# Krabbens/edge-diffusion-tts

Hardware: AMD Instinct MI355X
Metric: mel-frames/sec (whole node), 4-step DDIM, hidden=160 L=4, B=256 T=512 (higher is better)
Workload: dtype f32

## Files before the change

edge-diffusion-tts_amd/csrc/edtts_device.h:

```cpp
#pragma once
#include <hip/hip_runtime.h>
#include <stdint.h>
#include <type_traits>

#if !defined(EDTTS_EXPERIMENTS) && (                                                                                               \
    defined(EDTTS_ABLATE_QKVSTORES) || defined(EDTTS_ABLATE_KVLOADS) || defined(EDTTS_DIAG) || defined(EDTTS_KV2) ||                \
    defined(EDTTS_H_DMA) || defined(EDTTS_SPLITLOAD) || defined(EDTTS_STAMPS) || defined(EDTTS_DS_ABL) ||                           \
    defined(EDTTS_FAST_BUILD) || defined(EDTTS_W2) || defined(EDTTS_WAVELOG) || defined(EDTTS_PIN_MASK) || defined(EDTTS_HANDOVER) || defined(EDTTS_DS_BURST) || defined(EDTTS16_MFMA_SUM) || defined(EDTTS_DS_STAMPS) || defined(EDTTS_TAIL_RING2) || defined(EDTTS_RB) || defined(EDTTS_WMAX) ||        \
    defined(EDTTS_STAMP_THREAD) || defined(EDTTS_STAMP_HEAD) ||                                                                     \
    defined(EDTTS16_ABLATE_BARRIER) || defined(EDTTS16_ABLATE_DMA) || defined(EDTTS16_PHASES) || defined(EDTTS16_NF) ||             \
    defined(EDTTS16_W1) || defined(EDTTS16_QLDS) || defined(EDTTS16_KVDEPTH) || defined(EDTTS16_IMG) || defined(EDTTS16_HP) ||      \
    defined(EDTTS16_EVEN_STEPS))
#error "tuning / ablation / diagnostic / measured-and-rejected variant switches are scratch-only: add -DEDTTS_EXPERIMENTS"
#endif

#ifndef EDTTS_PIN_MASK
#define EDTTS_PIN_MASK 0x4
#endif
#ifndef EDTTS_W2
#define EDTTS_W2 0
#endif
#if EDTTS_W2
#define EDTTS_PIN_ACC(x) asm volatile("" : "+v"(x))
#else
#define EDTTS_PIN_ACC(x) asm volatile("" : "+a"(x))
#endif
typedef float f4 __attribute__((ext_vector_type(4)));
typedef float f2 __attribute__((ext_vector_type(2)));

#define EDTTS_MFMA(a, b, c) __builtin_amdgcn_mfma_f32_16x16x4f32((a), (b), (c), 0, 0, 0)
#define EDTTS_DEV __device__ __forceinline__

#ifdef EDTTS_STAMPS
#define STAMP_SEL_HEAD(sel) ((sel) & 0xff)
#define STAMPX(p, i, sel) do { if ((p) && (int)blockIdx.x == ((sel) >> 16) && (int)threadIdx.x == 64 * (((sel) >> 8) & 0xff)) (p)[i] = __builtin_amdgcn_s_memtime(); } while (0)
#else
#define STAMPX(p, i, sel) do { } while (0)
#endif

namespace edtts {

constexpr int kCtxWaves = 4;

template <int H_, int HEADS_, int MEL_, int NF_ = 2>
struct Cfg {
  static constexpr int H = H_, HEADS = HEADS_, MEL = MEL_, NF = NF_;
  static constexpr int WF = 16 * NF;
  static constexpr int QT = NF >= 2 ? 2 : 1;
  static constexpr int NHALF = NF / QT;
  static constexpr int DH = H / HEADS;
  static constexpr int DFULL = DH / 16;
  static constexpr int DREM = DH % 16;
  static constexpr int DT = (DH + 15) / 16;
  static constexpr int DHP = DT * 16;
  static constexpr int HT = H / 16;
  static constexpr int MT = MEL / 16;
  static constexpr int R = H / 2, RT = R / 16;
  static constexpr int VR = (HEADS - 1) * DH + DHP;
#ifndef EDTTS_WMAX
#define EDTTS_WMAX 2
#endif
  static constexpr int WAVES0 = (HT * NF * 4 <= 160) ? 4 : 2;
  static constexpr int WAVES = NF == 1 ? 1 : (WAVES0 < EDTTS_WMAX ? WAVES0 : EDTTS_WMAX);
  static constexpr bool Q_IN_LDS = !(EDTTS_W2 && NF == 2) && WF * H * 4 * 2 <= 40 * 1024;
  static constexpr int THREADS = 64 * WAVES;
  static constexpr bool DEFER = EDTTS_W2 && NF == 2 && H == 160;
  static constexpr int OHEAD_BYTES = DFULL * NF * 1024 + (DREM ? NF * 512 : 0);
  static_assert(NF == 1 || NF == 2 || NF == 4, "frame tiles per wave");
  static_assert(H % 32 == 0 && MEL % 16 == 0 && H % HEADS == 0, "dims");
  static_assert(DREM == 0 || DREM == 8, "head_dim % 16 must be 0 or 8");
};

EDTTS_DEV f4 splat(float v) { return f4{v, v, v, v}; }
EDTTS_DEV f4 ldg4(const float* p) { return *reinterpret_cast<const f4*>(p); }
EDTTS_DEV f2 ldg2(const float* p) { return *reinterpret_cast<const f2*>(p); }
EDTTS_DEV void stg4(float* p, f4 v) { *reinterpret_cast<f4*>(p) = v; }
EDTTS_DEV f4 ldg4_sbase(const float* base, unsigned byte_off) {
  return *reinterpret_cast<const f4*>(reinterpret_cast<const char*>(base) + byte_off);
}
EDTTS_DEV f2 ldg2_sbase(const float* base, unsigned byte_off) {
  return *reinterpret_cast<const f2*>(reinterpret_cast<const char*>(base) + byte_off);
}

template <int NT, int NF>
EDTTS_DEV void dma_tile_to_lds(const float* src, int ld, f4* lds_wave) {
  typedef __attribute__((address_space(3))) char* lds_char_t;
  const unsigned base = __builtin_amdgcn_readfirstlane((unsigned)(size_t)(lds_char_t)(char*)lds_wave);
#pragma unroll
  for (int nt = 0; nt < NT; ++nt)
#pragma unroll
    for (int ft = 0; ft < NF; ++ft) {
      const float* p = src + 16 * nt + (size_t)ft * 16 * ld;
      asm volatile("s_mov_b32 m0, %1\n\ts_nop 0\n\tglobal_load_lds_dwordx4 %0, off" ::"v"(p), "s"(base + (unsigned)(nt * NF + ft) * 1024u) : "m0", "memory");
    }
}

typedef unsigned u4v __attribute__((ext_vector_type(4)));
typedef unsigned u2v __attribute__((ext_vector_type(2)));
EDTTS_DEV __amdgpu_buffer_rsrc_t make_rsrc(const void* base) {
  return __builtin_amdgcn_make_buffer_rsrc(const_cast<void*>(base), 0, 0xFFFFFFFF, 0x00020000);
}
EDTTS_DEV f4 bufld4(__amdgpu_buffer_rsrc_t r, unsigned voff, unsigned soff) {
  return __builtin_bit_cast(f4, __builtin_amdgcn_raw_buffer_load_b128(r, voff, soff, 0));
}
EDTTS_DEV f2 bufld2(__amdgpu_buffer_rsrc_t r, unsigned voff, unsigned soff) {
  return __builtin_bit_cast(f2, __builtin_amdgcn_raw_buffer_load_b64(r, voff, soff, 0));
}

EDTTS_DEV float sqrt_rn(float x) { return (float)sqrt((double)x); }
EDTTS_DEV float div_rn(float a, float b) { return (float)((double)a / (double)b); }

EDTTS_DEV float group_sum(float v) {
  unsigned u = __float_as_uint(v);
  auto a = __builtin_amdgcn_permlane16_swap(u, u, false, false);
  v = __uint_as_float(a[0]) + __uint_as_float(a[1]);
  u = __float_as_uint(v);
  auto b = __builtin_amdgcn_permlane32_swap(u, u, false, false);
  return __uint_as_float(b[0]) + __uint_as_float(b[1]);
}
EDTTS_DEV float group_max(float v) {
  unsigned u = __float_as_uint(v);
  auto a = __builtin_amdgcn_permlane16_swap(u, u, false, false);
  v = fmaxf(__uint_as_float(a[0]), __uint_as_float(a[1]));
  u = __float_as_uint(v);
  auto b = __builtin_amdgcn_permlane32_swap(u, u, false, false);
  return fmaxf(__uint_as_float(b[0]), __uint_as_float(b[1]));
}
EDTTS_DEV float hsum(f4 v) { return (v[0] + v[1]) + (v[2] + v[3]); }
EDTTS_DEV float hmax(f4 v) { return fmaxf(fmaxf(v[0], v[1]), fmaxf(v[2], v[3])); }

#ifndef EDTTS_RB
#define EDTTS_RB 2
#endif
constexpr int kRefillBurst = EDTTS_RB;
template <int RN>
struct FragRing {
  static constexpr int RN_ = RN;
  __amdgpu_buffer_rsrc_t rs;
  unsigned soff;
  unsigned voff;
  f4 r[RN];
  EDTTS_DEV f4 frag(int i) const {
    return bufld4(rs, voff, soff + (unsigned)i * 1024u);
  }
  EDTTS_DEV void prime(const float* base, int lane) {
    rs = make_rsrc(base);
    soff = 0;
    voff = (unsigned)lane * 16u;
#pragma unroll
    for (int i = 0; i < RN; ++i) r[i] = frag(i);
  }
  EDTTS_DEV const f4& at(int i) const { return r[i % RN]; }
  EDTTS_DEV void refill(int lo, int hi) {
#pragma unroll
    for (int i = lo; i < hi; ++i) r[i % RN] = frag(i + RN);
    __builtin_amdgcn_sched_barrier(0);
  }
  template <int N>
  EDTTS_DEV void refill_after(int i) {
    constexpr int B = kRefillBurst < RN ? kRefillBurst : RN;
    if ((i + 1) % B == 0) refill(i + 1 - B, i + 1);
    else if (i == N - 1) refill(N - N % B, N);
  }
  EDTTS_DEV void advance(int n) { soff += (unsigned)n * 1024u; }
};

template <int KT, int RN, int NF>
EDTTS_DEV void gemm_phase(FragRing<RN>& ring, const f4 (&in)[KT][NF], f4 (&acc)[NF]) {
  static_assert(KT % RN == 0, "phase length must be a multiple of the ring size");
  constexpr bool SPLIT = NF < 4;
  f4 b[NF];
  if (SPLIT) {
#pragma unroll
    for (int ft = 0; ft < NF; ++ft) b[ft] = splat(0.f);
  }
#pragma unroll
  for (int kt = 0; kt < KT; ++kt) {
    const f4& a = ring.at(kt);
#pragma unroll
    for (int r = 0; r < 4; ++r)
#pragma unroll
      for (int ft = 0; ft < NF; ++ft) {
        if (SPLIT && (kt & 1)) b[ft] = EDTTS_MFMA(a[r], in[kt][ft][r], b[ft]);
        else acc[ft] = EDTTS_MFMA(a[r], in[kt][ft][r], acc[ft]);
      }
    ring.template refill_after<KT>(kt);
  }
  if (SPLIT) {
#pragma unroll
    for (int ft = 0; ft < NF; ++ft) acc[ft] += b[ft];
  }
  ring.advance(KT);
}

template <int KT, int RN, int NF>
EDTTS_DEV void gemm_phase_pair(FragRing<RN>& ring, const f4 (&in)[KT][NF], f4 (&a)[NF], f4 (&b)[NF]) {
  static_assert((2 * KT) % RN == 0, "phase length must be a multiple of the ring size");
#pragma unroll
  for (int kt = 0; kt < KT; ++kt) {
    const f4& fa = ring.at(2 * kt);
    const f4& fb = ring.at(2 * kt + 1);
#pragma unroll
    for (int r = 0; r < 4; ++r) {
#pragma unroll
      for (int ft = 0; ft < NF; ++ft) a[ft] = EDTTS_MFMA(fa[r], in[kt][ft][r], a[ft]);
#pragma unroll
      for (int ft = 0; ft < NF; ++ft) b[ft] = EDTTS_MFMA(fb[r], in[kt][ft][r], b[ft]);
    }
    ring.template refill_after<2 * KT>(2 * kt);
    ring.template refill_after<2 * KT>(2 * kt + 1);
  }
  ring.advance(2 * KT);
}

template <int NT, int RN, int NF, int NR = 4>
EDTTS_DEV void ktile_phase(FragRing<RN>& ring, const f4 (&in)[NF], f4 (&acc)[NT][NF]) {
  static_assert(NT % RN == 0, "phase length must be a multiple of the ring size");
  constexpr int STEP = NF < 4 ? 2 : 1;
#pragma unroll
  for (int nt = 0; nt < NT; nt += STEP) {
#pragma unroll
    for (int r = 0; r < NR; ++r)
#pragma unroll
      for (int u = 0; u < STEP; ++u)
        if (nt + u < NT) {
          const f4& fa = ring.at(nt + u);
#pragma unroll
          for (int ft = 0; ft < NF; ++ft) acc[nt + u][ft] = EDTTS_MFMA(fa[r], in[ft][r], acc[nt + u][ft]);
        }
#pragma unroll
    for (int u = 0; u < STEP; ++u)
      if (nt + u < NT) ring.template refill_after<NT>(nt + u);
  }
  ring.advance(NT);
}

template <int NT, int NF>
EDTTS_DEV void rms_norm_tile(const f4 (&x)[NT][NF], const float* __restrict__ w, const float* __restrict__ mod, int g,
                             f4 (&y)[NT][NF]) {
  constexpr int N = NT * 16;
  float rs[NF];
#pragma unroll
  for (int ft = 0; ft < NF; ++ft) {
    float ss = 0.f;
#pragma unroll
    for (int t = 0; t < NT; ++t) ss += hsum(x[t][ft] * x[t][ft]);
    rs[ft] = rsqrtf(group_sum(ss) * (1.0f / N) + 1e-6f);
  }
#pragma unroll
  for (int t = 0; t < NT; ++t) {
    const f4 wv = ldg4(w + 16 * t + 4 * g);
    f4 sc = splat(1.f), sh = splat(0.f);
    if (mod != nullptr) {
      sc = ldg4(mod + 16 * t + 4 * g);
      sh = ldg4(mod + N + 16 * t + 4 * g);
    }
#pragma unroll
    for (int ft = 0; ft < NF; ++ft) {
      f4 a = x[t][ft] * rs[ft] * wv;
// ... 658 lines not shown
```

edge-diffusion-tts_amd/csrc/edtts_kernels.hip:

```cpp
#include <hip/hip_runtime.h>
#include <math.h>
#include <stdarg.h>
#include <stdlib.h>
#include <stdio.h>
#include <string.h>

#include "../../include/edtts.h"
#include "edtts_device.h"

using namespace edtts;

static thread_local char g_err[512] = "";
static int fail(int code, const char* fmt, ...) __attribute__((format(printf, 2, 3)));
static int fail(int code, const char* fmt, ...) {
  va_list ap;
  va_start(ap, fmt);
  vsnprintf(g_err, sizeof(g_err), fmt, ap);
  va_end(ap);
  return code;
}
#define HIP_TRY(expr)                                                                                   \
  do {                                                                                                  \
    hipError_t e_ = (expr);                                                                             \
    if (e_ != hipSuccess) return fail(EDTTS_ERR_HIP, "%s failed: %s", #expr, hipGetErrorString(e_));    \
// ... 318 lines not shown
  const int64_t* step_idx;
  int use_host, host_has_step;
  int t_host[kMaxHostRows], step_host[kMaxHostRows];
  int H, L, n_step;
  const float *freqs, *t1T, *t1b, *t3T, *t3b, *step;
  const float* blob;
  unsigned ada1T[kMaxLayers], ada1b[kMaxLayers], ada3T[kMaxLayers], ada3b[kMaxLayers];
  float* cond;
  float* tcond;
  unsigned* err;
};
__global__ __launch_bounds__(256) void k_cond_mlp(CondArgs a) {
  extern __shared__ float sm[];
  float* e = sm;
  float* u = sm + a.H;
  const int row = blockIdx.x, tid = threadIdx.x, H = a.H, half = H / 2;
  const float tf = a.use_host ? (float)a.t_host[row] : (float)a.t[row];
  for (int j = tid; j < H; j += blockDim.x) {
    const float arg = tf * a.freqs[j < half ? j : j - half];
    e[j] = j < half ? sinf(arg) : cosf(arg);
  }
  __syncthreads();
  for (int n = tid; n < H; n += blockDim.x) {
    float acc = a.t1b[n];
#pragma unroll 8
    for (int k = 0; k < H; ++k) acc = fmaf(e[k], a.t1T[(size_t)k * H + n], acc);
    u[n] = 0.5f * acc * (1.0f + erff(acc * 0.70710678118654752440f));
  }
  __syncthreads();
  long sidx = -1;
  if (a.use_host ? a.host_has_step : (a.step_idx != nullptr)) {
    sidx = a.use_host ? (long)a.step_host[row] : (long)a.step_idx[row];
    if (sidx < 0 || sidx >= a.n_step) {
      if (tid == 0) atomicOr(a.err, (unsigned)EDTTS_IDX_STEP);
      sidx = sidx < 0 ? 0 : a.n_step - 1;
    }
  }
  for (int n = tid; n < H; n += blockDim.x) {
    float acc = a.t3b[n];
#pragma unroll 8
    for (int k = 0; k < H; ++k) acc = fmaf(u[k], a.t3T[(size_t)k * H + n], acc);
    if (sidx >= 0) acc += a.step[(size_t)sidx * H + n];
    a.tcond[(size_t)row * H + n] = acc;
  }
}
__global__ __launch_bounds__(256) void k_cond_ada(CondArgs a) {
  extern __shared__ float sm[];
  const int row = blockIdx.x, lw = blockIdx.y, l = lw >> 1, which = lw & 1, H = a.H;
  for (int k = threadIdx.x; k < H; k += blockDim.x) sm[k] = a.tcond[(size_t)row * H + k];
  __syncthreads();
  const float* WT = a.blob + (which ? a.ada3T[l] : a.ada1T[l]);
  const float* bb = a.blob + (which ? a.ada3b[l] : a.ada1b[l]);
  float* out = a.cond + (((size_t)row * a.L + l) * 2 + which) * 2 * H;
  for (int n = blockIdx.z * blockDim.x + threadIdx.x; n < 2 * H; n += gridDim.z * blockDim.x) {
    float acc = bb[n];
#pragma unroll 8
    for (int k = 0; k < H; ++k) acc = fmaf(sm[k], WT[(size_t)k * 2 * H + n], acc);
    out[n] = n < H ? 1.0f + acc : acc;
  }
}

struct KArgs {
  int B, T, Tp, S, Sp, window, max_pos, max_cpos, n_tok, SD, L;
  const float* x;
  float* h;
  const float *q, *k, *vT;
  float *q_out, *k_out, *vT_out;
  float *kc, *vcT;
  const void* unused_[3];
  const int64_t* sem_idx;
  const float* sem_feat;
  const float* cond;
  int cond_bstride;
  int layer;
  int ffn_tiles;
  int diag_skip;
  unsigned long long* stamps;
  const float *tok, *semp, *semp_b, *cpe, *inp, *inp_b, *pe;
  const float *n1w, *proj_b, *n2w, *n3w, *up_b, *down_b, *fnw, *fnb, *outp_b;
  const float* stream;
  float *eps, *x_prev, *x0;
  float c_s1m, c_sab, c_sabp, c_dir;
  float p_coef1, p_coef2, p_sd;
  const float* noise;
  unsigned long long seed;
  unsigned long long philox_base;
  unsigned step;
  LmsCoef lms;
  VpredCoef vp;
  const float* v_uncond;
  const float *h_new, *h_old;
  float *x0_hist, *x0_all;
  const int64_t *t_len, *s_len;
  int t_dbl;
};

EDTTS_DEV int utt_len_of(int64_t v, int full, bool dbl) {
  const int hi = dbl ? full >> 1 : full;
  const int n = v < 1 ? 1 : (v > hi ? hi : (int)v);
  return dbl ? 2 * n : n;
}
EDTTS_DEV int utt_len(const int64_t* len, int b, int full, bool dbl = false) {
  if (len == nullptr) return full;
  return utt_len_of(len[__builtin_amdgcn_readfirstlane(b)], full, dbl);
}
EDTTS_DEV int utt_len_lane(const int64_t* len, int b, int full, bool dbl = false) {
  return len == nullptr ? full : utt_len_of(len[b], full, dbl);
}
EDTTS_DEV int live_end(int n) { return (n + 31) & ~31; }

EDTTS_DEV int remap_block(int bid, int nblk) {
  const int q = nblk >> 3, r = nblk & 7, xcd = bid & 7, idx = bid >> 3;
  const int base = xcd < r ? xcd * (q + 1) : r * (q + 1) + (xcd - r) * q;
  return base + idx;
}

struct TileId {
  int b, m0;
  bool valid;
};
EDTTS_DEV TileId wave_tile(int B, int Tp, int waves_per_block, int wave_frames) {
  const int wave = __builtin_amdgcn_readfirstlane(threadIdx.x >> 6);
  const int tpu = Tp / wave_frames;
  int w = remap_block(blockIdx.x, gridDim.x) * waves_per_block + wave;
  TileId t;
  t.valid = w < B * tpu;
  w = t.valid ? w : B * tpu - 1;
  t.b = w / tpu;
  t.m0 = (w - t.b * tpu) * wave_frames;
  return t;
}

#ifndef EDTTS_TAIL_RING2
#define EDTTS_TAIL_RING2 1
#endif
template <class C>
EDTTS_DEV void qkv_tail(WStream<C>& ring0, const f4 (&hn)[C::HT][C::NF], const KArgs& a, int b, int m0, int lane) {
  constexpr int NF = C::NF;
  static_assert(C::HT % 2 == 0, "hidden must be a multiple of 32 (n-tile pairs)");
#if EDTTS_TAIL_RING2
  constexpr int RN0 = WStream<C>::RN_;
  static_assert((2 * C::HT) % (2 * RN0) == 0, "a pair phase must be a whole number of turns of the doubled ring");
  FragRing<2 * RN0> ring;
  ring.rs = ring0.rs; ring.soff = ring0.soff; ring.voff = ring0.voff;
#pragma unroll
  for (int i = 0; i < RN0; ++i) ring.r[i] = ring0.at(i);
#pragma unroll
  for (int i = RN0; i < 2 * RN0; ++i) ring.r[i] = ring.frag(i);
  __builtin_amdgcn_sched_barrier(0);
#else
  WStream<C>& ring = ring0;
#endif
  const int fq = lane & 15, g = lane >> 4;
  const size_t rowbase = (size_t)b * a.Tp + m0 + fq;
#pragma unroll
  for (int which = 0; which < 3; ++which) {
    for (int nt = 0; nt < C::HT; nt += 2) {
      f4 acc[2][NF];
#pragma unroll
      for (int ft = 0; ft < NF; ++ft) acc[0][ft] = acc[1][ft] = splat(0.f);
      gemm_phase_pair<C::HT>(ring, hn, acc[0], acc[1]);
#ifdef EDTTS_ABLATE_QKVSTORES
      if (a.T > 0) continue;
#endif
#pragma unroll
      for (int u = 0; u < 2; ++u) {
        if (which < 2) {
          float* dst = (which == 0 ? a.q_out : a.k_out) + rowbase * C::H + 16 * (nt + u) + 4 * g;
#pragma unroll
          for (int ft = 0; ft < NF; ++ft) {
            __builtin_nontemporal_store(acc[u][ft], reinterpret_cast<f4*>(dst + (size_t)ft * 16 * C::H));
          }
        } else {
          float* dst = a.vT_out + ((size_t)b * C::VR + 16 * (nt + u) + 4 * g) * a.Tp + m0 + fq;
#pragma unroll
          for (int r = 0; r < 4; ++r)
#pragma unroll
            for (int ft = 0; ft < NF; ++ft) {
              __builtin_nontemporal_store(acc[u][ft][r], dst + (size_t)r * a.Tp + 16 * ft);
            }
        }
      }
    }
  }
}

template <class C>
__global__ __launch_bounds__(C::THREADS) void k_prologue(KArgs a) {
  constexpr int NF = C::NF;
  const TileId tl = wave_tile(a.B, a.Tp, C::WAVES, C::WF);
  if (!tl.valid) return;
  const int lane = threadIdx.x & 63, fq = lane & 15, g = lane >> 4;
  const int b = tl.b, m0 = tl.m0;
  const int Tb = utt_len(a.t_len, b, a.T, a.t_dbl);
  if (m0 >= live_end(Tb)) return;
  WStream<C> ring;
  ring.prime(a.stream, lane);
  f4 xin[C::MT][NF];
#pragma unroll
  for (int ft = 0; ft < NF; ++ft) {
    const int f = m0 + 16 * ft + fq;
#pragma unroll
    for (int t = 0; t < C::MT; ++t)
      xin[t][ft] = f < Tb ? ldg4(a.x + ((size_t)b * a.T + f) * C::MEL + 16 * t + 4 * g) : splat(0.f);
  }
  f4 h[C::HT][NF];
#pragma unroll
  for (int nt = 0; nt < C::HT; ++nt) {
    const f4 bias = ldg4(a.inp_b + 16 * nt + 4 * g);
#pragma unroll
    for (int ft = 0; ft < NF; ++ft) h[nt][ft] = bias;
  }
  {
    constexpr int N = C::HT * C::MT;
    static_assert(N % WStream<C>::RN_ == 0 && C::HT % 2 == 0, "in_proj must be a whole number of ring turns");
#pragma unroll
    for (int nt = 0; nt < C::HT; nt += 2)
#pragma unroll
      for (int kt = 0; kt < C::MT; ++kt) {
        const int i = nt * C::MT + 2 * kt;
        const f4& fa = ring.at(i);
        const f4& fb = ring.at(i + 1);
#pragma unroll
        for (int r = 0; r < 4; ++r) {
#pragma unroll
          for (int ft = 0; ft < NF; ++ft) h[nt][ft] = EDTTS_MFMA(fa[r], xin[kt][ft][r], h[nt][ft]);
#pragma unroll
          for (int ft = 0; ft < NF; ++ft) h[nt + 1][ft] = EDTTS_MFMA(fb[r], xin[kt][ft][r], h[nt + 1][ft]);
        }
        ring.template refill_after<N>(i);
        ring.template refill_after<N>(i + 1);
      }
    ring.advance(N);
  }
#pragma unroll
  for (int ft = 0; ft < NF; ++ft) {
    int f = m0 + 16 * ft + fq;
    f = f < a.max_pos ? f : a.max_pos - 1;
#pragma unroll
    for (int nt = 0; nt < C::HT; ++nt) h[nt][ft] += ldg4(a.pe + (size_t)f * C::H + 16 * nt + 4 * g);
  }
  {
    float* hp = a.h + ((size_t)b * a.Tp + m0 + fq) * C::H + 4 * g;
#pragma unroll
    for (int nt = 0; nt < C::HT; ++nt)
#pragma unroll
      for (int ft = 0; ft < NF; ++ft) stg4(hp + 16 * nt + (size_t)ft * 16 * C::H, h[nt][ft]);
  }
  f4 hn[C::HT][NF];
  const float* mod = a.cond + (size_t)b * a.cond_bstride;
  rms_norm_tile<C::HT, NF>(h, a.n1w, mod, g, hn);
  qkv_tail<C>(ring, hn, a, b, m0, lane);
}

enum { TAIL_QKV = 0, TAIL_EPS = 1, TAIL_DDIM = 2, TAIL_DDPM = 3, TAIL_LMS = 4, TAIL_VPRED = 5 };

template <int TAIL>
EDTTS_DEV void tail_apply(const KArgs& a, size_t idx, f4 ev) {
  if (TAIL == TAIL_EPS) {
    stg4(a.eps + idx, ev);
  } else if (TAIL == TAIL_LMS) {
    const f4 xv = ldg4(a.x + idx);
    f4 hn = splat(0.f), ho = splat(0.f);
    if (a.lms.mode >= 2) hn = ldg4(a.h_new + idx);
    if (a.lms.mode >= 3) ho = ldg4(a.h_old + idx);
    f4 x0, xn;
#pragma unroll
    for (int r = 0; r < 4; ++r) {
      float v0, vn;
      lms_elem(xv[r], ev[r], hn[r], ho[r], a.lms, v0, vn);
      x0[r] = v0;
      xn[r] = vn;
    }
    stg4(a.x0_hist + idx, x0);
    if (a.x0_all) stg4(a.x0_all + idx, x0);
    stg4(a.x_prev + idx, xn);
  } else if (TAIL == TAIL_VPRED) {
    const bool guided = a.v_uncond != nullptr;
    const f4 xv = ldg4(a.x + idx);
    const f4 vu = ldg4((guided ? a.v_uncond : a.x) + idx);
    f4 v, xn;
#pragma unroll
    for (int r = 0; r < 4; ++r) v[r] = guided ? cfg_combine(ev[r], vu[r], a.vp.cfg) : ev[r];
#pragma unroll
    for (int r = 0; r < 4; ++r) xn[r] = vpred_elem(xv[r], v[r], a.vp);
    stg4(a.x_prev + idx, xn);
  } else if (TAIL == TAIL_DDPM) {
    const f4 xv = ldg4(a.x + idx);
    const f4 nz = a.noise ? ldg4(a.noise + idx) : philox_normal4(a.seed, a.step, (a.philox_base + idx) >> 2);
    const DdpmCoef cf{a.p_coef1, a.p_coef2, a.p_sd};
    f4 xp;
#pragma unroll
    for (int r = 0; r < 4; ++r) xp[r] = ddpm_elem(xv[r], ev[r], nz[r], cf);
    stg4(a.x_prev + idx, xp);
  } else {
    const f4 xv = ldg4(a.x + idx);
    f4 x0, xp;
#pragma unroll
    for (int r = 0; r < 4; ++r) {
      float v0, vp;
      ddim_elem(xv[r], ev[r], a.c_s1m, a.c_sab, a.c_sabp, a.c_dir, v0, vp);
      x0[r] = v0;
      xp[r] = vp;
    }
    stg4(a.x0 + idx, x0);
    stg4(a.x_prev + idx, xp);
  }
}
template <int TAIL>
EDTTS_DEV void tail_zero(const KArgs& a, size_t idx) {
  const f4 z = splat(0.f);
  if (TAIL == TAIL_EPS) {
    stg4(a.eps + idx, z);
  } else if (TAIL == TAIL_LMS) {
    stg4(a.x0_hist + idx, z);
    if (a.x0_all) stg4(a.x0_all + idx, z);
    stg4(a.x_prev + idx, z);
  } else if (TAIL == TAIL_DDIM) {
    stg4(a.x0 + idx, z);
    stg4(a.x_prev + idx, z);
  } else {
    stg4(a.x_prev + idx, z);
  }
}
template <int TAIL>
EDTTS_DEV void tail_store(const KArgs& a, int f, int Tb, size_t idx, f4 ev) {
  if (f < Tb) tail_apply<TAIL>(a, idx, ev);
  else tail_zero<TAIL>(a, idx);
}

struct QGlobal {
  __amdgpu_buffer_rsrc_t rs;
  unsigned v4, v2;
  int H;
  EDTTS_DEV QGlobal(const float* row_m0, int H_, int fq, int g) : rs(make_rsrc(row_m0)), v4((unsigned)(fq * H_ + 4 * g) * 4u), v2((unsigned)(fq * H_ + 2 * g) * 4u), H(H_) {}
  EDTTS_DEV f4 q4(int ft, int col) const { return bufld4(rs, v4, (unsigned)(ft * 16 * H + col) * 4u); }
  EDTTS_DEV f2 q2(int ft, int col) const { return bufld2(rs, v2, (unsigned)(ft * 16 * H + col) * 4u); }
};
struct QLds {
  const float* b4;
  const float* b2;
  int ld;
  EDTTS_DEV QLds(const float* tile, int ld_, int fq, int g) : b4(tile + fq * ld_ + 4 * g), b2(tile + fq * ld_ + 2 * g), ld(ld_) {}
  EDTTS_DEV f4 q4(int ft, int col) const { return *reinterpret_cast<const f4*>(b4 + ft * 16 * ld + col); }
  EDTTS_DEV f2 q2(int ft, int col) const { return *reinterpret_cast<const f2*>(b2 + ft * 16 * ld + col); }
};

template <class C, int TAIL>
EDTTS_DEV void layer_tile(const KArgs& a, float* smem, int wave, int lane, int b, int m0, int Tb, int Sb) {
  constexpr int NF = C::NF;
  const int fq = lane & 15, g = lane >> 4;
  f4* const stash = reinterpret_cast<f4*>(smem) + (size_t)wave * C::HT * NF * 64 + lane;
  char* const obuf = reinterpret_cast<char*>(smem) + (size_t)wave * C::HT * NF * 1024;
  static_assert(!C::DEFER || C::HEADS * C::OHEAD_BYTES <= C::HT * NF * 1024, "attention outputs must fit the wave's parking place");
  constexpr int QLDS = C::H;
  float* qtile = smem + (size_t)C::WAVES * C::HT * NF * 256 + (size_t)wave * C::WF * QLDS;
  const size_t rowbase = (size_t)b * a.Tp + m0 + fq;

  STAMPX(a.stamps, 0, a.diag_skip);
  WStream<C> ring;
  ring.prime(a.stream, lane);

  f4 h[C::HT][NF];
  float* const hp = a.h + rowbase * C::H + 4 * g;
  auto park_h = [&]() {
#pragma unroll
    for (int nt = 0; nt < C::HT; ++nt)
#pragma unroll
      for (int ft = 0; ft < NF; ++ft) stash[(nt * NF + ft) * 64] = h[nt][ft];
  };
  auto add_parked_h = [&]() {
#pragma unroll
    for (int nt = 0; nt < C::HT; ++nt)
#pragma unroll
      for (int ft = 0; ft < NF; ++ft) h[nt][ft] += stash[(nt * NF + ft) * 64];
  };
#ifdef EDTTS_DIAG
#define DIAG_ON(bit) (!(a.diag_skip & (bit)))
#else
#define DIAG_ON(bit) true
#endif
  {
#ifndef EDTTS_H_DMA
#define EDTTS_H_DMA 0
#endif
#if EDTTS_H_DMA
    dma_tile_to_lds<C::HT, NF>(hp, C::H, reinterpret_cast<f4*>(smem) + (size_t)wave * C::HT * NF * 64);
#else
    if constexpr (!C::DEFER) {
#pragma unroll
      for (int nt = 0; nt < C::HT; ++nt)
#pragma unroll
        for (int ft = 0; ft < NF; ++ft) h[nt][ft] = ldg4(hp + 16 * nt + (size_t)ft * 16 * C::H);
      park_h();
    }
#endif
    auto init_proj_bias = [&]() {
#pragma unroll
      for (int nt = 0; nt < C::HT; ++nt) {
        const f4 pb = ldg4(a.proj_b + 16 * nt + 4 * g);
#pragma unroll
        for (int ft = 0; ft < NF; ++ft) h[nt][ft] = pb;
      }
    };
    if constexpr (!C::DEFER) init_proj_bias();
    if (DIAG_ON(1)) {
      QGlobal ql(a.q + ((size_t)b * a.Tp + m0) * C::H, C::H, fq, g);
      attention_fused<C, true, C::DEFER ? O_DEFER : O_FUSED>(ql, a.k + (size_t)b * a.Tp * C::H, a.vT + (size_t)b * C::VR * a.Tp, a.Tp, Tb, a.window, m0,
                               lane, ring, h, obuf, init_proj_bias, a.stamps ? a.stamps + 8 : nullptr, a.diag_skip);
    }
    if constexpr (C::DEFER) {
#pragma unroll
      for (int nt = 0; nt < C::HT; ++nt)
#pragma unroll
        for (int ft = 0; ft < NF; ++ft) h[nt][ft] += ldg4(hp + 16 * nt + (size_t)ft * 16 * C::H);
    } else {
      add_parked_h();
    }
    STAMPX(a.stamps, 1, a.diag_skip);
  }
  if (DIAG_ON(2)) {
    {
      f4 hn[C::HT][NF];
      rms_norm_tile<C::HT, NF>(h, a.n2w, nullptr, g, hn);
      if constexpr (C::DEFER) {
#pragma unroll
        for (int nt = 0; nt < C::HT; ++nt)
#pragma unroll
          for (int ft = 0; ft < NF; ++ft) stg4(hp + 16 * nt + (size_t)ft * 16 * C::H, h[nt][ft]);
      } else {
        park_h();
      }
      for (int nt = 0; nt < C::HT; nt += 2) {
        f4 acc[2][NF];
#pragma unroll
        for (int ft = 0; ft < NF; ++ft) acc[0][ft] = acc[1][ft] = splat(0.f);
        gemm_phase_pair<C::HT>(ring, hn, acc[0], acc[1]);
#pragma unroll
        for (int u = 0; u < 2; ++u)
#pragma unroll
          for (int ft = 0; ft < NF; ++ft) {
            if (C::Q_IN_LDS) stg4(qtile + (16 * ft + fq) * QLDS + 16 * (nt + u) + 4 * g, acc[u][ft]);
            else stg4(const_cast<float*>(a.q) + (rowbase + 16 * ft) * C::H + 16 * (nt + u) + 4 * g, acc[u][ft]);
          }
      }
    }
    STAMPX(a.stamps, 2, a.diag_skip);
    auto zero_h = [&]() {
#pragma unroll
      for (int nt = 0; nt < C::HT; ++nt)
#pragma unroll
        for (int ft = 0; ft < NF; ++ft) h[nt][ft] = splat(0.f);
    };
    if constexpr (!C::DEFER) zero_h();
    if constexpr (C::Q_IN_LDS) {
      QLds ql(qtile, QLDS, fq, g);
      attention_fused<C, false, C::DEFER ? O_DEFER : O_FUSED>(ql, a.kc + (size_t)b * a.Sp * C::H, a.vcT + (size_t)b * C::VR * a.Sp, a.Sp, Sb, -1, m0, lane,
                                ring, h, obuf, zero_h, a.stamps ? a.stamps + 40 : nullptr, a.diag_skip);
    } else {
      QGlobal ql(a.q + ((size_t)b * a.Tp + m0) * C::H, C::H, fq, g);
      attention_fused<C, false, C::DEFER ? O_DEFER : O_FUSED>(ql, a.kc + (size_t)b * a.Sp * C::H, a.vcT + (size_t)b * C::VR * a.Sp, a.Sp, Sb, -1, m0, lane,
                                ring, h, obuf, zero_h);
    }
    if constexpr (C::DEFER) {
#pragma unroll
      for (int nt = 0; nt < C::HT; ++nt)
#pragma unroll
        for (int ft = 0; ft < NF; ++ft) h[nt][ft] += ldg4(hp + 16 * nt + (size_t)ft * 16 * C::H);
    } else {
      add_parked_h();
    }
    STAMPX(a.stamps, 3, a.diag_skip);
  }
  if (DIAG_ON(4)) {
    f4 hn[C::HT][NF];
    const float* mod = a.cond + (size_t)b * a.cond_bstride + ((size_t)a.layer * 2 + 1) * 2 * C::H;
    rms_norm_tile<C::HT, NF>(h, a.n3w, mod, g, hn);
    park_h();
#pragma unroll
    for (int nt = 0; nt < C::HT; ++nt) {
      const f4 db = ldg4(a.down_b + 16 * nt + 4 * g);
#pragma unroll
      for (int ft = 0; ft < NF; ++ft) h[nt][ft] = db;
    }
    for (int j = 0; j < a.ffn_tiles; ++j) {
      const f4 vb = ldg4(a.up_b + 32 * j + 4 * g), gb = ldg4(a.up_b + 32 * j + 16 + 4 * g);
      f4 v[NF], gt[NF], act[NF];
#pragma unroll
      for (int ft = 0; ft < NF; ++ft) v[ft] = gt[ft] = splat(0.f);
      gemm_phase_pair<C::HT>(ring, hn, v, gt);
      __builtin_amdgcn_sched_barrier(0);
#pragma unroll
      for (int ft = 0; ft < NF; ++ft) act[ft] = swiglu_tile(v[ft], gt[ft], vb, gb);
      __builtin_amdgcn_sched_barrier(0);
      ktile_phase<C::HT>(ring, act, h);
    }
    add_parked_h();
    STAMPX(a.stamps, 4, a.diag_skip);
  }
  if (!DIAG_ON(8)) return;
  if (TAIL == TAIL_QKV) {
    {
      float* hp = a.h + rowbase * C::H + 4 * g;
#pragma unroll
      for (int nt = 0; nt < C::HT; ++nt)
#pragma unroll
        for (int ft = 0; ft < NF; ++ft) stg4(hp + 16 * nt + (size_t)ft * 16 * C::H, h[nt][ft]);
    }
    const float* mod = a.cond + (size_t)b * a.cond_bstride + ((size_t)(a.layer + 1) * 2) * 2 * C::H;
    rms_norm_tile<C::HT, NF>(h, a.n1w, mod, g, h);
    qkv_tail<C>(ring, h, a, b, m0, lane);
  } else {
    f4 hn[C::HT][NF];
    layer_norm_tile<C::HT, NF>(h, a.fnw, a.fnb, g, hn);
#pragma unroll
    for (int nt = 0; nt < C::MT; ++nt) {
      const f4 ob = ldg4(a.outp_b + 16 * nt + 4 * g);
      f4 e[NF];
#pragma unroll
      for (int ft = 0; ft < NF; ++ft) e[ft] = splat(0.f);
      gemm_phase<C::HT>(ring, hn, e);
#pragma unroll
      for (int ft = 0; ft < NF; ++ft) {
        const int f = m0 + 16 * ft + fq;
        if (f >= a.T) continue;
        const size_t idx = ((size_t)b * a.T + f) * C::MEL + 16 * nt + 4 * g;
        tail_store<TAIL>(a, f, Tb, idx, e[ft] + ob);
      }
    }
  }
  STAMPX(a.stamps, 5, a.diag_skip);
#ifdef EDTTS_STAMPS
  asm volatile("s_waitcnt vmcnt(0)" ::: "memory");
#endif
  STAMPX(a.stamps, 6, a.diag_skip);
}

template <class C, int TAIL>
EDTTS_DEV void tail_zero_tile(const KArgs& a, int b, int m0, int lane) {
  const int fq = lane & 15, g = lane >> 4;
#pragma unroll
  for (int ft = 0; ft < C::NF; ++ft) {
    const int f = m0 + 16 * ft + fq;
    if (f >= a.T) continue;
#pragma unroll
    for (int nt = 0; nt < C::MT; ++nt) tail_zero<TAIL>(a, ((size_t)b * a.T + f) * C::MEL + 16 * nt + 4 * g);
  }
}
template <class C, int TAIL>
__global__ __launch_bounds__(C::THREADS, C::DEFER ? 2 : 1) void k_layer(KArgs a) {
  extern __shared__ __attribute__((aligned(16))) float smem[];
  const int lane = threadIdx.x & 63;
  const int wave = __builtin_amdgcn_readfirstlane(threadIdx.x >> 6);
  const TileId tl = wave_tile(a.B, a.Tp, C::WAVES, C::WF);
  if (!tl.valid) return;
  const int Tb = utt_len(a.t_len, tl.b, a.T, a.t_dbl);
  if (tl.m0 >= live_end(Tb)) {
    if constexpr (TAIL != TAIL_QKV) tail_zero_tile<C, TAIL>(a, tl.b, tl.m0, lane);
    return;
  }
  const int Sb = utt_len(a.s_len, tl.b, a.S);
#ifdef EDTTS_WAVELOG
  const unsigned long long wl_r0 = __builtin_amdgcn_s_memrealtime(), wl_c0 = __builtin_amdgcn_s_memtime();
#endif
  layer_tile<C, TAIL>(a, smem, wave, lane, tl.b, tl.m0, Tb, Sb);
#ifdef EDTTS_WAVELOG
  if (a.stamps && lane == 0) {
    asm volatile("s_waitcnt vmcnt(0)" ::: "memory");
    unsigned long long* p = a.stamps + 6 * ((size_t)a.diag_skip + (size_t)tl.b * (a.Tp / C::WF) + tl.m0 / C::WF);
    p[0] = wl_r0; p[1] = wl_c0; p[2] = __builtin_amdgcn_s_memrealtime(); p[3] = __builtin_amdgcn_s_memtime();
    p[4] = __builtin_amdgcn_s_getreg((31 << 11) | 4);
    p[5] = __builtin_amdgcn_s_getreg((31 << 11) | 20);
  }
#endif
}

#include "edtts_coop.h"
#include "edtts_bf16.h"
#include "edtts_melpost.h"

struct CtxArgs {
  int B, S, Sp, L, SD, n_tok, max_cpos;
  const int64_t* sem_idx;
  const float* sem_feat;
  const float *tok, *semp, *semp_b, *cpe;
  const float* blob;
  unsigned kvd[kMaxLayers], kvn[kMaxLayers], kvu[kMaxLayers];
  float *kc, *vcT;
  unsigned* err;
  const float* stream16;
  const int64_t* s_len;
};
template <class C>
__global__ __launch_bounds__(64 * kCtxWaves) void k_ctx(CtxArgs a) {
  const TileId tl = wave_tile(a.B, a.Sp, kCtxWaves, 32);
  if (!tl.valid) return;
  const int lane = threadIdx.x & 63, fq = lane & 15, g = lane >> 4;
  const int b = tl.b, m0 = tl.m0;
  const int Sb = utt_len(a.s_len, b, a.S);
  if (m0 >= live_end(Sb)) return;
  f4 ctx[C::HT][2];
  if (a.sem_feat != nullptr) {
    const int KT = a.SD / 16;
    const f4* wp = reinterpret_cast<const f4*>(a.semp) + lane;
#pragma unroll
    for (int nt = 0; nt < C::HT; ++nt) ctx[nt][0] = ctx[nt][1] = ldg4(a.semp_b + 16 * nt + 4 * g);
    for (int kt = 0; kt < KT; ++kt) {
      f4 xin[2];
#pragma unroll
      for (int ft = 0; ft < 2; ++ft) {
        const int s = m0 + 16 * ft + fq;
        xin[ft] = s < Sb ? ldg4(a.sem_feat + ((size_t)b * a.S + s) * a.SD + 16 * kt + 4 * g) : splat(0.f);
      }
#pragma unroll
      for (int nt = 0; nt < C::HT; ++nt) {
        const f4 w = wp[(nt * KT + kt) * 64];
#pragma unroll
        for (int r = 0; r < 4; ++r) {
          ctx[nt][0] = EDTTS_MFMA(w[r], xin[0][r], ctx[nt][0]);
          ctx[nt][1] = EDTTS_MFMA(w[r], xin[1][r], ctx[nt][1]);
        }
      }
    }
  } else {
#pragma unroll
    for (int ft = 0; ft < 2; ++ft) {
      const int s = m0 + 16 * ft + fq;
      long tk = s < Sb ? (long)a.sem_idx[(size_t)b * a.S + s] : 0;
      if (tk < 0 || tk >= a.n_tok) {
        atomicOr(a.err, (unsigned)EDTTS_IDX_SEM);
        tk = tk < 0 ? 0 : a.n_tok - 1;
      }
      const float* row = a.tok + (size_t)tk * C::H + 4 * g;
#pragma unroll
      for (int nt = 0; nt < C::HT; ++nt) ctx[nt][ft] = ldg4(row + 16 * nt);
    }
  }
#pragma unroll
  for (int ft = 0; ft < 2; ++ft) {
    int s = m0 + 16 * ft + fq;
    s = s < a.max_cpos ? s : a.max_cpos - 1;
    const float* row = a.cpe + (size_t)s * C::H + 4 * g;
#pragma unroll
    for (int nt = 0; nt < C::HT; ++nt) ctx[nt][ft] += ldg4(row + 16 * nt);
  }
  const int lpb = (a.L + (int)gridDim.y - 1) / (int)gridDim.y;
  const int l_end = ((int)blockIdx.y + 1) * lpb < a.L ? ((int)blockIdx.y + 1) * lpb : a.L;
  for (int l = (int)blockIdx.y * lpb; l < l_end; ++l) {
    f4 c[C::RT][2];
    {
      FragRing<C::HT> ring;
      ring.prime(a.blob + a.kvd[l], lane);
#pragma unroll
      for (int nt = 0; nt < C::RT; ++nt) {
        c[nt][0] = c[nt][1] = splat(0.f);
        gemm_phase<C::HT>(ring, ctx, c[nt]);
      }
    }
    f4 cn[C::RT][2];
    rms_norm_tile<C::RT, 2>(c, a.blob + a.kvn[l], nullptr, g, cn);
    FragRing<C::RT> ring;
    ring.prime(a.blob + a.kvu[l], lane);
    float* kdst = a.kc + (((size_t)l * a.B + b) * a.Sp + m0 + fq) * C::H + 4 * g;
    float* vdst = a.vcT + (((size_t)l * a.B + b) * C::VR + 4 * g) * a.Sp + m0 + fq;
    for (int nt = 0; nt < 2 * C::HT; ++nt) {
      f4 acc[2] = {splat(0.f), splat(0.f)};
      gemm_phase<C::RT>(ring, cn, acc);
      if (nt < C::HT) {
        stg4(kdst + 16 * nt, acc[0]);
        stg4(kdst + 16 * nt + 16 * C::H, acc[1]);
      } else {
        float* d = vdst + (size_t)(16 * (nt - C::HT)) * a.Sp;
#pragma unroll
        for (int r = 0; r < 4; ++r) {
          d[(size_t)r * a.Sp] = acc[0][r];
          d[(size_t)r * a.Sp + 16] = acc[1][r];
        }
      }
    }
  }
}

template <class C>
__global__ __launch_bounds__(C::THREADS, 1) void k_ctx16(CtxArgs a) {
  using namespace edtts16;
  extern __shared__ __attribute__((aligned(16))) f4 ring_lds_ctx16[];
  constexpr int RT = C::R / 16, RK = C::R / 32, KT = C::KT;
  static_assert(C::NF == 2 && C::R % 32 == 0 && 2 * KT == C::PH && C::PH % (2 * RK) == 0, "context kernel geometry");
  constexpr int PPP = C::PH / (2 * RK);
  static_assert(C::HEADS % PPP == 0, "K heads and V heads do not share a phase");
  const TileId tl = wave_tile(a.B, a.Sp, C::WAVES, 32);
  const bool valid = tl.valid;
  const int lane = threadIdx.x & 63, fq = lane & 15, g = lane >> 4;
  const int b = tl.b, m0 = tl.m0;
  const int Sb = utt_len(a.s_len, b, a.S);
  LdsRing<C> ring;
  ring.start(a.stream16, ring_lds_ctx16, __builtin_amdgcn_readfirstlane(threadIdx.x >> 6), lane);
  f4 ctx[C::HT][2];
  if (a.sem_feat != nullptr) {
    const int SKT = a.SD / 16;
    const f4* wp = reinterpret_cast<const f4*>(a.semp) + lane;
#pragma unroll
    for (int nt = 0; nt < C::HT; ++nt) ctx[nt][0] = ctx[nt][1] = ldg4(a.semp_b + 16 * nt + 4 * g);
    for (int kt = 0; kt < SKT; ++kt) {
      f4 xin[2];
#pragma unroll
      for (int ft = 0; ft < 2; ++ft) {
        const int s = m0 + 16 * ft + fq;
        xin[ft] = s < Sb ? ldg4(a.sem_feat + ((size_t)b * a.S + s) * a.SD + 16 * kt + 4 * g) : splat(0.f);
      }
#pragma unroll
      for (int nt = 0; nt < C::HT; ++nt) {
        const f4 w = wp[(nt * SKT + kt) * 64];
#pragma unroll
        for (int r = 0; r < 4; ++r) {
          ctx[nt][0] = EDTTS_MFMA(w[r], xin[0][r], ctx[nt][0]);
          ctx[nt][1] = EDTTS_MFMA(w[r], xin[1][r], ctx[nt][1]);
        }
      }
    }
  } else {
#pragma unroll
    for (int ft = 0; ft < 2; ++ft) {
      const int s = m0 + 16 * ft + fq;
      long tk = s < Sb ? (long)a.sem_idx[(size_t)b * a.S + s] : 0;
      if (tk < 0 || tk >= a.n_tok) {
        atomicOr(a.err, (unsigned)EDTTS_IDX_SEM);
        tk = tk < 0 ? 0 : a.n_tok - 1;
      }
      const float* row = a.tok + (size_t)tk * C::H + 4 * g;
#pragma unroll
      for (int nt = 0; nt < C::HT; ++nt) ctx[nt][ft] = ldg4(row + 16 * nt);
    }
  }
#pragma unroll
  for (int ft = 0; ft < 2; ++ft) {
    int s = m0 + 16 * ft + fq;
    s = s < a.max_cpos ? s : a.max_cpos - 1;
    const float* row = a.cpe + (size_t)s * C::H + 4 * g;
#pragma unroll
    for (int nt = 0; nt < C::HT; ++nt) ctx[nt][ft] += ldg4(row + 16 * nt);
  }
  bf8 xin[KT][2];
#pragma unroll
  for (int kt = 0; kt < KT; ++kt)
#pragma unroll
    for (int ft = 0; ft < 2; ++ft) xin[kt][ft] = pack8(ctx[2 * kt][ft], ctx[2 * kt + 1][ft]);
  const size_t hstride = (size_t)32 * a.Sp;
  const int lpb = (a.L + (int)gridDim.y - 1) / (int)gridDim.y;
  const int l_end = ((int)blockIdx.y + 1) * lpb < a.L ? ((int)blockIdx.y + 1) * lpb : a.L;
  for (int l = (int)blockIdx.y * lpb; l < l_end; ++l) {
    f4 c[RT][2];
#pragma unroll
    for (int p = 0; p < RT / 2; ++p) {
      c[2 * p][0] = c[2 * p][1] = c[2 * p + 1][0] = c[2 * p + 1][1] = splat(0.f);
      gemm16_pair<KT, false>(ring, xin, c[2 * p], c[2 * p + 1]);
    }
    bf8 cn[RK][2];
    {
      float rs[2];
#pragma unroll
      for (int ft = 0; ft < 2; ++ft) {
        float ss = 0.f;
#pragma unroll
        for (int t = 0; t < RT; ++t) ss += hsum(c[t][ft] * c[t][ft]);
        rs[ft] = rsqrtf(group_sum(ss) * (1.0f / C::R) + 1e-6f);
      }
      const float* w = a.blob + a.kvn[l];
#pragma unroll
      for (int kt = 0; kt < RK; ++kt) {
        const f4 w0 = ldg4(w + 32 * kt + 4 * g), w1 = ldg4(w + 32 * kt + 16 + 4 * g);
#pragma unroll
        for (int ft = 0; ft < 2; ++ft) cn[kt][ft] = pack8(c[2 * kt][ft] * rs[ft] * w0, c[2 * kt + 1][ft] * rs[ft] * w1);
      }
    }
    __bf16* const kimg = reinterpret_cast<__bf16*>(a.kc) + ((size_t)l * a.B + b) * a.Sp * C::H;
    __bf16* const vimg = reinterpret_cast<__bf16*>(a.vcT) + ((size_t)l * a.B + b) * a.Sp * C::H;
    for (int ph = 0; ph < 2 * C::HEADS / PPP; ++ph) {
      const lds_cf4_t fr = phase_base(ring.acquire());
      f4 fg[C::PH];
#pragma unroll
      for (int i = 0; i < C::PH; ++i) fg[i] = fr[i * 64];
      __builtin_amdgcn_sched_barrier(0);
      const bool isv = ph >= C::HEADS / PPP;
#pragma unroll
      for (int pp = 0; pp < PPP; ++pp) {
        const int head = (isv ? ph - C::HEADS / PPP : ph) * PPP + pp;
        f4 acc[2][2] = {{splat(0.f), splat(0.f)}, {splat(0.f), splat(0.f)}};
        if (!isv) {
#pragma unroll
          for (int kt = 0; kt < RK; ++kt)
#pragma unroll
            for (int u = 0; u < 2; ++u)
#pragma unroll
              for (int ft = 0; ft < 2; ++ft)
                acc[u][ft] = EDTTS_MFMA16(as_bf8(fg[pp * 2 * RK + 2 * kt + u]), cn[kt][ft], acc[u][ft]);
          __bf16* d = kimg + head * hstride + (size_t)(m0 >> 4) * 512 + fq * 32 + 8 * g;
          if (valid)
#pragma unroll
            for (int ft = 0; ft < 2; ++ft) *reinterpret_cast<f4*>(d + ft * 512) = as_f4(pack8(acc[0][ft], acc[1][ft]));
        } else {
#pragma unroll
          for (int kt = 0; kt < RK; ++kt)
#pragma unroll
            for (int u = 0; u < 2; ++u)
#pragma unroll
              for (int ft = 0; ft < 2; ++ft)
                acc[u][ft] = EDTTS_MFMA16(cn[kt][ft], as_bf8(fg[pp * 2 * RK + 2 * kt + u]), acc[u][ft]);
          __bf16* d = vimg + head * hstride + (size_t)(m0 >> 5) * 1024 + fq * 32 + 8 * g;
          if (valid)
#pragma unroll
            for (int u = 0; u < 2; ++u) *reinterpret_cast<f4*>(d + u * 512) = as_f4(pack8(acc[u][0], acc[u][1]));
        }
      }
    }
  }
  ring.drain();
}


struct StepArgs {
  const float *alphas, *alpha_bar, *betas, *post_var;
  int n_table;
  const float *x, *eps, *noise;
  const int64_t *t, *t_prev;
  size_t n_per_batch;
  float eta;
  float *x_prev, *x0;
  int vec4;
// ... 2162 lines not shown
```

Before: 8.692 million.

## Use buffer stores/loads with scalar offsets and hoist tile loads ahead of GEMMs

Replaces global pointer-based stores and loads in the QKV tail, prologue, output tail and context KV kernel with raw buffer ops that use a per-tile resource descriptor plus scalar offsets. This cuts 64-bit address arithmetic and VGPR pressure. The prologue now issues the positional-embedding loads up front with the input loads, and the DDIM tail prefetches x before the layer norm. The context kernel primes the next layer's down-projection ring while the current up-projection runs. The trade-off is more live registers for the prefetched tiles, and buffer offsets are 32-bit, so very large tensors could overflow.

```diff
diff --git a/edge-diffusion-tts_amd/csrc/edtts_device.h b/edge-diffusion-tts_amd/csrc/edtts_device.h
--- a/edge-diffusion-tts_amd/csrc/edtts_device.h
+++ b/edge-diffusion-tts_amd/csrc/edtts_device.h
@@ -105,6 +105,18 @@
 }
 EDTTS_DEV f2 bufld2(__amdgpu_buffer_rsrc_t r, unsigned voff, unsigned soff) {
   return __builtin_bit_cast(f2, __builtin_amdgcn_raw_buffer_load_b64(r, voff, soff, 0));
+}
+EDTTS_DEV void bufst4_nt(__amdgpu_buffer_rsrc_t r, unsigned voff, unsigned soff, f4 v) {
+  __builtin_amdgcn_raw_buffer_store_b128(__builtin_bit_cast(u4v, v), r, voff, soff, 2);
+}
+EDTTS_DEV void bufst1_nt(__amdgpu_buffer_rsrc_t r, unsigned voff, unsigned soff, float v) {
+  __builtin_amdgcn_raw_buffer_store_b32(__builtin_bit_cast(unsigned, v), r, voff, soff, 2);
+}
+EDTTS_DEV void bufst4(__amdgpu_buffer_rsrc_t r, unsigned voff, unsigned soff, f4 v) {
+  __builtin_amdgcn_raw_buffer_store_b128(__builtin_bit_cast(u4v, v), r, voff, soff, 0);
+}
+EDTTS_DEV void bufst1(__amdgpu_buffer_rsrc_t r, unsigned voff, unsigned soff, float v) {
+  __builtin_amdgcn_raw_buffer_store_b32(__builtin_bit_cast(unsigned, v), r, voff, soff, 0);
 }
 
 EDTTS_DEV float sqrt_rn(float x) { return (float)sqrt((double)x); }
diff --git a/edge-diffusion-tts_amd/csrc/edtts_kernels.hip b/edge-diffusion-tts_amd/csrc/edtts_kernels.hip
--- a/edge-diffusion-tts_amd/csrc/edtts_kernels.hip
+++ b/edge-diffusion-tts_amd/csrc/edtts_kernels.hip
@@ -494,7 +494,12 @@
   WStream<C>& ring = ring0;
 #endif
   const int fq = lane & 15, g = lane >> 4;
-  const size_t rowbase = (size_t)b * a.Tp + m0 + fq;
+  const size_t row0 = (size_t)b * a.Tp + m0;
+  const __amdgpu_buffer_rsrc_t rs_q = make_rsrc(a.q_out + row0 * C::H), rs_k = make_rsrc(a.k_out + row0 * C::H);
+  const __amdgpu_buffer_rsrc_t rs_v = make_rsrc(a.vT_out + (size_t)b * C::VR * a.Tp + m0);
+  const unsigned voff_qk = (unsigned)(fq * C::H + 4 * g) * 4u;
+  const unsigned voff_v = (unsigned)(4 * g * a.Tp + fq) * 4u;
+  const unsigned tp4 = (unsigned)a.Tp * 4u;
 #pragma unroll
   for (int which = 0; which < 3; ++which) {
     for (int nt = 0; nt < C::HT; nt += 2) {
@@ -508,19 +513,15 @@
 #pragma unroll
       for (int u = 0; u < 2; ++u) {
         if (which < 2) {
-          float* dst = (which == 0 ? a.q_out : a.k_out) + rowbase * C::H + 16 * (nt + u) + 4 * g;
-#pragma unroll
-          for (int ft = 0; ft < NF; ++ft) {
-            __builtin_nontemporal_store(acc[u][ft], reinterpret_cast<f4*>(dst + (size_t)ft * 16 * C::H));
-          }
+#pragma unroll
+          for (int ft = 0; ft < NF; ++ft)
+            bufst4_nt(which == 0 ? rs_q : rs_k, voff_qk, (unsigned)(ft * 16 * C::H + 16 * (nt + u)) * 4u, acc[u][ft]);
         } else {
-          float* dst = a.vT_out + ((size_t)b * C::VR + 16 * (nt + u) + 4 * g) * a.Tp + m0 + fq;
+          const unsigned row = (unsigned)(16 * (nt + u)) * tp4;
 #pragma unroll
           for (int r = 0; r < 4; ++r)
 #pragma unroll
-            for (int ft = 0; ft < NF; ++ft) {
-              __builtin_nontemporal_store(acc[u][ft][r], dst + (size_t)r * a.Tp + 16 * ft);
-            }
+            for (int ft = 0; ft < NF; ++ft) bufst1_nt(rs_v, voff_v, row + (unsigned)r * tp4 + 64u * ft, acc[u][ft][r]);
         }
       }
     }
@@ -539,12 +540,26 @@
   WStream<C> ring;
   ring.prime(a.stream, lane);
   f4 xin[C::MT][NF];
-#pragma unroll
-  for (int ft = 0; ft < NF; ++ft) {
-    const int f = m0 + 16 * ft + fq;
-#pragma unroll
-    for (int t = 0; t < C::MT; ++t)
-      xin[t][ft] = f < Tb ? ldg4(a.x + ((size_t)b * a.T + f) * C::MEL + 16 * t + 4 * g) : splat(0.f);
+  f4 pe[C::HT][NF];
+  {
+    const __amdgpu_buffer_rsrc_t rs_x = make_rsrc(a.x + ((size_t)b * a.T + m0) * C::MEL), rs_pe = make_rsrc(a.pe);
+    const unsigned voff_x = (unsigned)(fq * C::MEL + 4 * g) * 4u;
+#pragma unroll
+    for (int ft = 0; ft < NF; ++ft) {
+      const int f = m0 + 16 * ft + fq;
+#pragma unroll
+      for (int t = 0; t < C::MT; ++t)
+        xin[t][ft] = f < Tb ? bufld4(rs_x, voff_x, (unsigned)(ft * 16 * C::MEL + 16 * t) * 4u) : splat(0.f);
+    }
+#pragma unroll
+    for (int ft = 0; ft < NF; ++ft) {
+      int f = m0 + 16 * ft + fq;
+      f = f < a.max_pos ? f : a.max_pos - 1;
+      const unsigned voff_pe = (unsigned)(f * C::H + 4 * g) * 4u;
+#pragma unroll
+      for (int nt = 0; nt < C::HT; ++nt) pe[nt][ft] = bufld4(rs_pe, voff_pe, (unsigned)(16 * nt) * 4u);
+    }
+    __builtin_amdgcn_sched_barrier(0);
   }
   f4 h[C::HT][NF];
 #pragma unroll
@@ -576,18 +591,16 @@
     ring.advance(N);
   }
 #pragma unroll
-  for (int ft = 0; ft < NF; ++ft) {
-    int f = m0 + 16 * ft + fq;
-    f = f < a.max_pos ? f : a.max_pos - 1;
-#pragma unroll
-    for (int nt = 0; nt < C::HT; ++nt) h[nt][ft] += ldg4(a.pe + (size_t)f * C::H + 16 * nt + 4 * g);
-  }
+  for (int ft = 0; ft < NF; ++ft)
+#pragma unroll
+    for (int nt = 0; nt < C::HT; ++nt) h[nt][ft] += pe[nt][ft];
   {
-    float* hp = a.h + ((size_t)b * a.Tp + m0 + fq) * C::H + 4 * g;
+    const __amdgpu_buffer_rsrc_t rs_h = make_rsrc(a.h + ((size_t)b * a.Tp + m0) * C::H);
+    const unsigned voff_h = (unsigned)(fq * C::H + 4 * g) * 4u;
 #pragma unroll
     for (int nt = 0; nt < C::HT; ++nt)
 #pragma unroll
-      for (int ft = 0; ft < NF; ++ft) stg4(hp + 16 * nt + (size_t)ft * 16 * C::H, h[nt][ft]);
+      for (int ft = 0; ft < NF; ++ft) bufst4(rs_h, voff_h, (unsigned)(16 * nt + ft * 16 * C::H) * 4u, h[nt][ft]);
   }
   f4 hn[C::HT][NF];
   const float* mod = a.cond + (size_t)b * a.cond_bstride;
@@ -596,6 +609,19 @@
 }
 
 enum { TAIL_QKV = 0, TAIL_EPS = 1, TAIL_DDIM = 2, TAIL_DDPM = 3, TAIL_LMS = 4, TAIL_VPRED = 5 };
+
+EDTTS_DEV void ddim_apply(const KArgs& a, size_t idx, f4 xv, f4 ev) {
+  f4 x0, xp;
+#pragma unroll
+  for (int r = 0; r < 4; ++r) {
+    float v0, vp;
+    ddim_elem(xv[r], ev[r], a.c_s1m, a.c_sab, a.c_sabp, a.c_dir, v0, vp);
+    x0[r] = v0;
+    xp[r] = vp;
+  }
+  stg4(a.x0 + idx, x0);
+  stg4(a.x_prev + idx, xp);
+}
 
 template <int TAIL>
 EDTTS_DEV void tail_apply(const KArgs& a, size_t idx, f4 ev) {
@@ -636,17 +662,7 @@
     for (int r = 0; r < 4; ++r) xp[r] = ddpm_elem(xv[r], ev[r], nz[r], cf);
     stg4(a.x_prev + idx, xp);
   } else {
-    const f4 xv = ldg4(a.x + idx);
-    f4 x0, xp;
-#pragma unroll
-    for (int r = 0; r < 4; ++r) {
-      float v0, vp;
-      ddim_elem(xv[r], ev[r], a.c_s1m, a.c_sab, a.c_sabp, a.c_dir, v0, vp);
-      x0[r] = v0;
-      xp[r] = vp;
-    }
-    stg4(a.x0 + idx, x0);
-    stg4(a.x_prev + idx, xp);
+    ddim_apply(a, idx, ldg4(a.x + idx), ev);
   }
 }
 template <int TAIL>
@@ -843,16 +859,28 @@
   if (!DIAG_ON(8)) return;
   if (TAIL == TAIL_QKV) {
     {
-      float* hp = a.h + rowbase * C::H + 4 * g;
+      const __amdgpu_buffer_rsrc_t rs_h = make_rsrc(a.h + ((size_t)b * a.Tp + m0) * C::H);
+      const unsigned voff_h = (unsigned)(fq * C::H + 4 * g) * 4u;
 #pragma unroll
       for (int nt = 0; nt < C::HT; ++nt)
 #pragma unroll
-        for (int ft = 0; ft < NF; ++ft) stg4(hp + 16 * nt + (size_t)ft * 16 * C::H, h[nt][ft]);
+        for (int ft = 0; ft < NF; ++ft) bufst4(rs_h, voff_h, (unsigned)(16 * nt + ft * 16 * C::H) * 4u, h[nt][ft]);
     }
     const float* mod = a.cond + (size_t)b * a.cond_bstride + ((size_t)(a.layer + 1) * 2) * 2 * C::H;
     rms_norm_tile<C::HT, NF>(h, a.n1w, mod, g, h);
     qkv_tail<C>(ring, h, a, b, m0, lane);
   } else {
+    f4 xt[TAIL == TAIL_DDIM ? C::MT : 1][NF];
+    if constexpr (TAIL == TAIL_DDIM) {
+#pragma unroll
+      for (int ft = 0; ft < NF; ++ft) {
+        const int f = m0 + 16 * ft + fq;
+#pragma unroll
+        for (int nt = 0; nt < C::MT; ++nt)
+          xt[nt][ft] = f < Tb ? ldg4(a.x + ((size_t)b * a.T + f) * C::MEL + 16 * nt + 4 * g) : splat(0.f);
+      }
+      __builtin_amdgcn_sched_barrier(0);
+    }
     f4 hn[C::HT][NF];
     layer_norm_tile<C::HT, NF>(h, a.fnw, a.fnb, g, hn);
 #pragma unroll
@@ -867,7 +895,12 @@
         const int f = m0 + 16 * ft + fq;
         if (f >= a.T) continue;
         const size_t idx = ((size_t)b * a.T + f) * C::MEL + 16 * nt + 4 * g;
-        tail_store<TAIL>(a, f, Tb, idx, e[ft] + ob);
+        if constexpr (TAIL == TAIL_DDIM) {
+          if (f < Tb) ddim_apply(a, idx, xt[nt][ft], e[ft] + ob);
+          else tail_zero<TAIL>(a, idx);
+        } else {
+          tail_store<TAIL>(a, f, Tb, idx, e[ft] + ob);
+        }
       }
     }
   }
@@ -988,35 +1021,38 @@
   }
   const int lpb = (a.L + (int)gridDim.y - 1) / (int)gridDim.y;
   const int l_end = ((int)blockIdx.y + 1) * lpb < a.L ? ((int)blockIdx.y + 1) * lpb : a.L;
-  for (int l = (int)blockIdx.y * lpb; l < l_end; ++l) {
+  const int l_begin = (int)blockIdx.y * lpb;
+  const unsigned voff_k = (unsigned)(fq * C::H + 4 * g) * 4u, voff_v = (unsigned)(4 * g * a.Sp + fq) * 4u, sp4 = (unsigned)a.Sp * 4u;
+  FragRing<C::HT> ring_d;
+  if (l_begin < l_end) ring_d.prime(a.blob + a.kvd[l_begin], lane);
+  for (int l = l_begin; l < l_end; ++l) {
+    FragRing<C::RT> ring;
+    ring.prime(a.blob + a.kvu[l], lane);
+    __builtin_amdgcn_sched_barrier(0);
     f4 c[C::RT][2];
-    {
-      FragRing<C::HT> ring;
-      ring.prime(a.blob + a.kvd[l], lane);
-#pragma unroll
-      for (int nt = 0; nt < C::RT; ++nt) {
-        c[nt][0] = c[nt][1] = splat(0.f);
-        gemm_phase<C::HT>(ring, ctx, c[nt]);
-      }
+#pragma unroll
+    for (int nt = 0; nt < C::RT; ++nt) {
+      c[nt][0] = c[nt][1] = splat(0.f);
+      gemm_phase<C::HT>(ring_d, ctx, c[nt]);
     }
     f4 cn[C::RT][2];
     rms_norm_tile<C::RT, 2>(c, a.blob + a.kvn[l], nullptr, g, cn);
-    FragRing<C::RT> ring;
-    ring.prime(a.blob + a.kvu[l], lane);
-    float* kdst = a.kc + (((size_t)l * a.B + b) * a.Sp + m0 + fq) * C::H + 4 * g;
-    float* vdst = a.vcT + (((size_t)l * a.B + b) * C::VR + 4 * g) * a.Sp + m0 + fq;
+    if (l + 1 < l_end) ring_d.prime(a.blob + a.kvd[l + 1], lane);
+    __builtin_amdgcn_sched_barrier(0);
+    const __amdgpu_buffer_rsrc_t rs_kc = make_rsrc(a.kc + (((size_t)l * a.B + b) * a.Sp + m0) * C::H);
+    const __amdgpu_buffer_rsrc_t rs_vc = make_rsrc(a.vcT + ((size_t)l * a.B + b) * C::VR * a.Sp + m0);
     for (int nt = 0; nt < 2 * C::HT; ++nt) {
       f4 acc[2] = {splat(0.f), splat(0.f)};
       gemm_phase<C::RT>(ring, cn, acc);
       if (nt < C::HT) {
-        stg4(kdst + 16 * nt, acc[0]);
-        stg4(kdst + 16 * nt + 16 * C::H, acc[1]);
+        bufst4(rs_kc, voff_k, (unsigned)(16 * nt) * 4u, acc[0]);
+        bufst4(rs_kc, voff_k, (unsigned)(16 * nt + 16 * C::H) * 4u, acc[1]);
       } else {
-        float* d = vdst + (size_t)(16 * (nt - C::HT)) * a.Sp;
+        const unsigned row = (unsigned)(16 * (nt - C::HT)) * sp4;
 #pragma unroll
         for (int r = 0; r < 4; ++r) {
-          d[(size_t)r * a.Sp] = acc[0][r];
-          d[(size_t)r * a.Sp + 16] = acc[1][r];
+          bufst1(rs_vc, voff_v, row + (unsigned)r * sp4, acc[0][r]);
+          bufst1(rs_vc, voff_v, row + (unsigned)r * sp4 + 64u, acc[1][r]);
         }
       }
     }
```

New measurement: 8.747 million, median of 6. Within noise of the previous version (+0.6%).
